# yxtay/glove-tensorflow

Measured on AMD Instinct MI355X. Metric: co-occurrence nonzeros/sec, higher is better.
Workload: dtype f32; 1 GPU; zipf_v400k_d300; V=400000, d=300, optimizer=Adagrad, batch_size_per_gpu=1048576, global_batch=1048576, nnz_per_gpu=25000000, chunk_cap=32, parallelism=single GPU, index=dealt

## Files before the change

### glove-tensorflow_amd/csrc/glove_epoch.hip

```cpp
#include "glove_common.h"

#include <type_traits>

namespace glove {

constexpr int kCsThreads = 256;
constexpr int kCsWaves = kCsThreads / 64;
constexpr int kCsMaxDigits = 2048;
constexpr int kCsMaxBits = 11;

struct CsGeom {
    int64_t n;
    int ntiles;
    int nd[2], db[2];
    int stride;
    uint32_t *count, *offs;
    uint32_t *tot;
};

template <int E, class Job>
__global__ __launch_bounds__(kCsThreads) void csort_hist(Job job, CsGeom g)
{
    __shared__ int hist[kCsMaxDigits];
    const int side = blockIdx.y, nd = g.nd[side], db = g.db[side];
// ... 7 lines not shown
#pragma unroll
        for (int j = 0; j < E; ++j) {
            const int64_t i = base + j * 64 + lane;
            if (i < g.n) { walk[j * kCsThreads + threadIdx.x] = job.position(side, i); cnt = j + 1; }
        }
        int j = 0;
        uint32_t x = cnt > 0 ? walk[threadIdx.x] : 0u;
        while (j < cnt) {
            x = job.seat_once(x);
            if (job.seated(x)) {
                walk[j * kCsThreads + threadIdx.x] = x;
                ++j;
                if (j < cnt) x = walk[j * kCsThreads + threadIdx.x];
            }
        }
    }
#pragma unroll 4
    for (int j = 0; j < E; ++j) {
        const int64_t i = base + j * 64 + lane;
        const bool valid = i < g.n;
        int digit = 0;
        if (Job::kSeats) { if (valid) digit = job.digit_of_seat(side, i, walk[j * kCsThreads + threadIdx.x]); }
        else if (valid) digit = job.digit(side, i);
        const unsigned long long peers = digit_peers(digit, db, valid);
        if (valid && lane == __ffsll((long long)peers) - 1) atomicAdd(&hist[digit], __popcll(peers));
    }
    __syncthreads();
    uint32_t *out = g.count + (size_t)side * g.stride * g.ntiles + blockIdx.x;
    for (int i = threadIdx.x; i < nd; i += kCsThreads) out[(size_t)i * g.ntiles] = (uint32_t)hist[i];
}

__device__ inline int block_excl_scan(int v, int *wtot , int &total)
{
    const int lane = threadIdx.x & 63, wave = threadIdx.x >> 6;
    int incl = v;
#pragma unroll
    for (int dlt = 1; dlt < 64; dlt <<= 1) {
        const int o = __shfl_up(incl, dlt, 64);
        if (lane >= dlt) incl += o;
    }
    __syncthreads();
    if (lane == 63) wtot[wave] = incl;
    __syncthreads();
    int start = incl - v;
    total = 0;
#pragma unroll
    for (int wv = 0; wv < kCsWaves; ++wv) {
        if (wv < wave) start += wtot[wv];
        total += wtot[wv];
    }
    return start;
}

__global__ __launch_bounds__(kCsThreads) void csort_scan(CsGeom g)
{
    __shared__ int wtot[kCsWaves];
    const int side = blockIdx.y, d = blockIdx.x;
    if (d >= g.nd[side]) return;
    const uint32_t *row = g.count + ((size_t)side * g.stride + d) * g.ntiles;
    uint32_t *out = g.offs + ((size_t)side * g.stride + d) * g.ntiles;
    constexpr int kPer = 8;
    int carry = 0;
    for (int base = 0; base < g.ntiles; base += kCsThreads * kPer) {
        int v[kPer], s = 0;
#pragma unroll
        for (int k = 0; k < kPer; ++k) {
            const int t = base + threadIdx.x * kPer + k;
            v[k] = t < g.ntiles ? (int)row[t] : 0;
            s += v[k];
        }
        int total;
        int run = carry + block_excl_scan(s, wtot, total);
#pragma unroll
        for (int k = 0; k < kPer; ++k) {
            const int t = base + threadIdx.x * kPer + k;
            if (t < g.ntiles) out[t] = (uint32_t)run;
            run += v[k];
        }
        carry += total;
    }
    if (threadIdx.x == 0) g.tot[(size_t)side * g.stride + d] = (uint32_t)carry;
}

template <int E, class Job>
__global__ __launch_bounds__(kCsThreads) void csort_scatter(Job job, CsGeom g)
{
    using Item = typename Job::Item;
    constexpr int T = kCsThreads * E;
    extern __shared__ __attribute__((aligned(16))) unsigned char cs_smem[];
    const int side = blockIdx.y, nd = g.nd[side], db = g.db[side];
    Item *stage = reinterpret_cast<Item *>(cs_smem);
    uint16_t *sdig = reinterpret_cast<uint16_t *>(stage + T);
    int *wcnt = reinterpret_cast<int *>(sdig + T);
    int *gbase = wcnt + kCsWaves * nd;
    int *tstart = gbase + nd;
    __shared__ int wtot[kCsWaves];
    const int lane = threadIdx.x & 63, wave = threadIdx.x >> 6;
    const int64_t tile0 = (int64_t)blockIdx.x * T;
    const int64_t base = tile0 + (int64_t)wave * (64 * E);
    Item it[E];
    int digit[E], rank[E];
#pragma unroll
    for (int j = 0; j < E; ++j) {
        const int64_t i = base + j * 64 + lane;
        digit[j] = 0;
        if (i < g.n) digit[j] = job.load(side, i, it[j]);
    }
    int *mine = wcnt + wave * nd;
    for (int i = lane; i < nd; i += 64) mine[i] = 0;
#pragma unroll
    for (int j = 0; j < E; ++j) {
        const bool valid = base + j * 64 + lane < g.n;
        const unsigned long long peers = digit_peers(digit[j], db, valid);
        const int leader = valid ? __ffsll((long long)peers) - 1 : lane;
        int before = 0;
        if (valid && lane == leader) before = atomicAdd(&mine[digit[j]], __popcll(peers));
        before = __shfl(before, leader, 64);
        rank[j] = before + __popcll(peers & ((1ull << lane) - 1ull));
    }
    __syncthreads();
    constexpr int kPer = kCsMaxDigits / kCsThreads;
    {
        const uint32_t *tot = g.tot + (size_t)side * g.stride;
        const uint32_t *offs = g.offs + (size_t)side * g.stride * g.ntiles + blockIdx.x;
        int tile_n[kPer], all_n[kPer], st = 0, sa = 0;
#pragma unroll
        for (int k = 0; k < kPer; ++k) {
            const int d = threadIdx.x * kPer + k;
            tile_n[k] = all_n[k] = 0;
            if (d < nd) {
                int run = 0;
#pragma unroll
                for (int wv = 0; wv < kCsWaves; ++wv) {
                    const int c = wcnt[wv * nd + d];
                    wcnt[wv * nd + d] = run;
                    run += c;
                }
                tile_n[k] = run;
                all_n[k] = (int)tot[d];
            }
            st += tile_n[k];
            sa += all_n[k];
        }
        int total;
        int ts = block_excl_scan(st, wtot, total);
        int ds = block_excl_scan(sa, wtot, total);
#pragma unroll
        for (int k = 0; k < kPer; ++k) {
            const int d = threadIdx.x * kPer + k;
            if (d < nd) {
                tstart[d] = ts;
                gbase[d] = ds + (int)offs[(size_t)d * g.ntiles] - ts;
            }
            ts += tile_n[k];
            ds += all_n[k];
        }
    }
    __syncthreads();
#pragma unroll
    for (int j = 0; j < E; ++j) {
        if (base + j * 64 + lane >= g.n) continue;
        const int lp = tstart[digit[j]] + mine[digit[j]] + rank[j];
        stage[lp] = it[j];
        sdig[lp] = (uint16_t)digit[j];
    }
    __syncthreads();
    const int64_t left = g.n - tile0;
    const int count = left < T ? (int)left : T;
#pragma unroll 4
    for (int k = 0; k < E; ++k) {
        const int lp = k * kCsThreads + threadIdx.x;
        if (lp >= count) break;
        job.store(side, (int64_t)(gbase[sdig[lp]] + lp), stage[lp]);
    }
}

struct CsWs {
    uint32_t *count, *offs, *tot;
    int ntiles, e;
    size_t bytes;
};

static int cs_e_for(int stride) { (void)stride; return 8; }

static CsWs carve_cs(void *ws, int64_t n, int stride)
{
    CsWs c;
    char *base = (char *)ws;
    size_t off = 0;
    auto take = [&](size_t bytes) { void *q = base + off; off += align_up(bytes, 256); return q; };
    c.e = cs_e_for(stride);
    const int64_t per_tile = (int64_t)kCsThreads * c.e;
    c.ntiles = (int)((n + per_tile - 1) / per_tile);
    if (c.ntiles < 1) c.ntiles = 1;
    c.count = (uint32_t *)take((size_t)2 * c.ntiles * stride * 4);
    c.offs = (uint32_t *)take((size_t)2 * c.ntiles * stride * 4);
    c.tot = (uint32_t *)take((size_t)2 * stride * 4);
    c.bytes = off;
    return c;
}

template <int E, class Job>
static int launch_cs_pass(const Job &job, const CsGeom &g, hipStream_t st)
{
    const size_t smem = (size_t)kCsThreads * E * (sizeof(typename Job::Item) + 2) + (size_t)(kCsWaves + 2) * g.stride * 4;
    hipError_t e = hipFuncSetAttribute(reinterpret_cast<const void *>(csort_scatter<E, Job>), hipFuncAttributeMaxDynamicSharedMemorySize, (int)smem);
    if (e != hipSuccess) return (int)e;
    hipLaunchKernelGGL((csort_hist<E, Job>), dim3(g.ntiles, 2), dim3(kCsThreads), 0, st, job, g);
    hipLaunchKernelGGL(csort_scan, dim3(g.stride, 2), dim3(kCsThreads), 0, st, g);
    hipLaunchKernelGGL((csort_scatter<E, Job>), dim3(g.ntiles, 2), dim3(kCsThreads), smem, st, job, g);
    return (int)hipGetLastError();
}

template <class Job>
static int run_cs_pass(const Job &job, const CsWs &c, int64_t n, const int (&db)[2], hipStream_t st)
{
    CsGeom g;
    g.n = n;
    g.ntiles = c.ntiles;
    for (int sd = 0; sd < 2; ++sd) { g.db[sd] = db[sd]; g.nd[sd] = 1 << db[sd]; }
    g.stride = g.nd[0] > g.nd[1] ? g.nd[0] : g.nd[1];
    g.count = c.count; g.offs = c.offs; g.tot = c.tot;
    return c.e == 16 ? launch_cs_pass<16, Job>(job, g, st) : launch_cs_pass<8, Job>(job, g, st);
}

static int ceil_log2_64(int64_t v)
{
    int b = 1;
    while (b < 62 && (1ll << b) < v) ++b;
    return b;
}

struct DealSide {
    const int32_t *id, *partner;
    const float *w, *y;
    const int32_t *link;
    int32_t *o_id, *o_partner;
    float *o_w, *o_y;
    int32_t *cache;
    int4 *tmp_pay;
    int32_t *tmp_batch;
};

struct DealItemLast { int32_t id, partner, w, y; };
struct DealItemMid { int32_t id, partner, w, y, batch; };

template <bool FIRST, bool LAST>
struct DealJob {
    DealSide s[2];
    uint64_t n;
    uint32_t B;
    int bits;
    uint4 key;
    int shift;
    uint32_t mask;
    int bshift;
    int nt;
    int cache8;
    using Item = typename std::conditional<LAST, DealItemLast, DealItemMid>::type;

    static constexpr bool kSeats = FIRST;
    __device__ uint32_t position(int side, int64_t i) const { return s[side].link ? (uint32_t)s[side].link[i] : (uint32_t)i; }
    __device__ uint32_t seat_once(uint32_t x) const { return feistel_once(x, bits, key); }
    __device__ bool seated(uint32_t x) const { return x < (uint32_t)n; }
    __device__ int digit_of_seat(int side, int64_t i, uint32_t seat) const
    {
        const int32_t batch = (int32_t)(bshift >= 0 ? seat >> bshift : seat / B);
        if (cache8) reinterpret_cast<uint8_t *>(s[side].cache)[i] = (uint8_t)batch; else s[side].cache[i] = batch;
        return (int)(((uint32_t)batch >> shift) & mask);
    }
    __device__ int digit(int side, int64_t i) const
    {
        if (FIRST) return digit_of_seat(side, i, feistel_walk(position(side, i), (uint32_t)n, bits, key));
        return (int)(((uint32_t)s[side].tmp_batch[i] >> shift) & mask);
    }
    __device__ int load(int side, int64_t i, Item &it) const
    {
        const DealSide &sd = s[side];
        int32_t batch;
        if (FIRST) {
            if (nt) {
                it.id = __builtin_nontemporal_load(sd.id + i); it.partner = __builtin_nontemporal_load(sd.partner + i);
                it.w = __float_as_int(__builtin_nontemporal_load(sd.w + i)); it.y = __float_as_int(__builtin_nontemporal_load(sd.y + i));
                batch = cache8 ? (int32_t)__builtin_nontemporal_load(reinterpret_cast<const uint8_t *>(sd.cache) + i) : __builtin_nontemporal_load(sd.cache + i);
            } else {
                it.id = sd.id[i]; it.partner = sd.partner[i];
                it.w = __float_as_int(sd.w[i]); it.y = __float_as_int(sd.y[i]);
                batch = cache8 ? (int32_t)reinterpret_cast<const uint8_t *>(sd.cache)[i] : sd.cache[i];
            }
        } else {
            const int4 v = sd.tmp_pay[i];
            it.id = v.x; it.partner = v.y; it.w = v.z; it.y = v.w;
            batch = sd.tmp_batch[i];
        }
        set_batch(it, batch);
        return (int)(((uint32_t)batch >> shift) & mask);
    }
    __device__ static void set_batch(DealItemLast &, int32_t) {}
    __device__ static void set_batch(DealItemMid &it, int32_t b) { it.batch = b; }
    __device__ void store(int side, int64_t dest, const DealItemLast &it) const
    {
        const DealSide &sd = s[side];
        if (nt) {
            __builtin_nontemporal_store(it.id, sd.o_id + dest); __builtin_nontemporal_store(it.partner, sd.o_partner + dest);
            __builtin_nontemporal_store(__int_as_float(it.w), sd.o_w + dest); __builtin_nontemporal_store(__int_as_float(it.y), sd.o_y + dest);
        } else {
            sd.o_id[dest] = it.id; sd.o_partner[dest] = it.partner;
            sd.o_w[dest] = __int_as_float(it.w); sd.o_y[dest] = __int_as_float(it.y);
        }
    }
    __device__ void store(int side, int64_t dest, const DealItemMid &it) const
    {
        const DealSide &sd = s[side];
        sd.tmp_pay[dest] = make_int4(it.id, it.partner, it.w, it.y);
        sd.tmp_batch[dest] = it.batch;
    }
};

struct DealPlan { int passes, db[2]; int64_t nb; };
static DealPlan deal_plan(int64_t n, int64_t B)
{
    DealPlan p;
    p.nb = (n + B - 1) / B;
    const int bits = ceil_log2_64(p.nb > 1 ? p.nb : 2);
    p.passes = bits <= kCsMaxBits ? 1 : 2;
    p.db[0] = p.passes == 1 ? bits : (bits + 1) / 2;
    p.db[1] = p.passes == 1 ? 0 : bits - p.db[0];
    return p;
}

struct DealWs { CsWs cs; int32_t *cache[2]; int4 *pay[2]; int32_t *batch[2]; size_t bytes; };
static DealWs carve_deal(void *ws, int64_t n, int64_t B)
{
    const DealPlan p = deal_plan(n, B);
    DealWs d;
    const int stride = 1 << (p.db[0] > p.db[1] ? p.db[0] : p.db[1]);
    d.cs = carve_cs(ws, n, stride);
    size_t off = d.cs.bytes;
    char *base = (char *)ws;
    auto take = [&](size_t bytes) { void *q = base + off; off += align_up(bytes, 256); return q; };
    for (int sd = 0; sd < 2; ++sd) {
        d.cache[sd] = (int32_t *)take((size_t)n * 4);
        d.pay[sd] = p.passes > 1 ? (int4 *)take((size_t)n * 16) : nullptr;
        d.batch[sd] = p.passes > 1 ? (int32_t *)take((size_t)n * 4) : nullptr;
    }
    d.bytes = off;
    return d;
}

struct MasterSide {
    const int32_t *major, *minor;
    uint32_t major_below, minor_below;
    const uint64_t *k_in; uint64_t *k_out;
    const int32_t *i_in; int32_t *i_out;
    int32_t *o_id, *o_partner, *o_perm;
    int shift;
    uint32_t mask;
};

template <bool FIRST, bool LAST>
struct MasterJob {
    MasterSide s[2];
    struct Item { uint64_t key; int32_t idx; };
    __device__ uint64_t key_of(int side, int64_t i) const
    {
        const MasterSide &sd = s[side];
        if (!FIRST) return sd.k_in[i];
        uint32_t a = (uint32_t)sd.major[i], b = (uint32_t)sd.minor[i];
        if (a >= sd.major_below) a = 0;
        if (b >= sd.minor_below) b = 0;
        return (uint64_t)a << 32 | b;
    }
    static constexpr bool kSeats = false;
    __device__ uint32_t position(int, int64_t) const { return 0u; }
    __device__ uint32_t seat_once(uint32_t x) const { return x; }
    __device__ bool seated(uint32_t) const { return true; }
    __device__ int digit_of_seat(int, int64_t, uint32_t) const { return 0; }
    __device__ int digit(int side, int64_t i) const { return (int)((uint32_t)(key_of(side, i) >> s[side].shift) & s[side].mask); }
    __device__ int load(int side, int64_t i, Item &it) const
    {
        it.key = key_of(side, i);
        it.idx = FIRST ? (int32_t)i : s[side].i_in[i];
        return (int)((uint32_t)(it.key >> s[side].shift) & s[side].mask);
    }
    __device__ void store(int side, int64_t dest, const Item &it) const
    {
        const MasterSide &sd = s[side];
        if (LAST) {
            sd.o_id[dest] = (int32_t)(it.key >> 32);
            sd.o_partner[dest] = (int32_t)(uint32_t)it.key;
            sd.o_perm[dest] = it.idx;
        } else {
            sd.k_out[dest] = it.key;
            sd.i_out[dest] = it.idx;
        }
    }
};

__global__ __launch_bounds__(kBlock) void masters_gather_kernel(const float *__restrict__ w, const float *__restrict__ y,
                                                                const int32_t *__restrict__ row, const int32_t *__restrict__ col,
                                                                uint32_t row_below, uint32_t col_below, int64_t n,
                                                                const int32_t *__restrict__ perm_r, const int32_t *__restrict__ perm_c,
                                                                float *__restrict__ w_r, float *__restrict__ y_r,
                                                                float *__restrict__ w_c, float *__restrict__ y_c,
                                                                int32_t *__restrict__ inv_r, int32_t *__restrict__ mapped)
{
    int bad = 0;
    for (int64_t k = (int64_t)blockIdx.x * kBlock + threadIdx.x; k < n; k += (int64_t)gridDim.x * kBlock) {
        const int32_t pr = perm_r[k], pc = perm_c[k];
        w_r[k] = w[pr]; y_r[k] = y[pr];
        w_c[k] = w[pc]; y_c[k] = y[pc];
        inv_r[pr] = (int32_t)k;
        bad += ((uint32_t)row[k] >= row_below) + ((uint32_t)col[k] >= col_below);
    }
    bad = wave_sum_int(bad);
    if (mapped && (threadIdx.x & 63) == 0 && bad) atomicAdd(mapped, bad);
}

__global__ __launch_bounds__(kBlock) void masters_link_kernel(const int32_t *__restrict__ perm_c, const int32_t *__restrict__ inv_r,
                                                              int64_t n, int32_t *__restrict__ link)
{
    for (int64_t q = (int64_t)blockIdx.x * kBlock + threadIdx.x; q < n; q += (int64_t)gridDim.x * kBlock) link[q] = inv_r[perm_c[q]];
}

struct MastersWs { CsWs cs; uint64_t *key[2][2]; int32_t *idx[2][2]; int32_t *perm[2]; int32_t *inv; size_t bytes; };
static MastersWs carve_masters(void *ws, int64_t n)
{
    MastersWs m;
    m.cs = carve_cs(ws, n, kCsMaxDigits);
    size_t off = m.cs.bytes;
    char *base = (char *)ws;
    auto take = [&](size_t bytes) { void *q = base + off; off += align_up(bytes, 256); return q; };
    const size_t nn = (size_t)(n > 0 ? n : 1);
    for (int sd = 0; sd < 2; ++sd)
        for (int i = 0; i < 2; ++i) {
            m.key[sd][i] = (uint64_t *)take(nn * 8);
            m.idx[sd][i] = (int32_t *)take(nn * 4);
        }
    for (int sd = 0; sd < 2; ++sd) m.perm[sd] = (int32_t *)take(nn * 4);
    m.inv = (int32_t *)take(nn * 4);
    m.bytes = off;
    return m;
}

static bool pairs_ok(const glove_pairs *p) { return p && p->id && p->partner && p->w && p->y; }

}

using namespace glove;

extern "C" {

size_t glove_masters_workspace_bytes(int64_t n)
{
    if (n < 0) return 0;
    return carve_masters(nullptr, n).bytes;
// ... 98 lines not shown
```

### glove-tensorflow_amd/csrc/glove_plan.hip

```cpp
#include "glove_common.h"

#include <cstring>

namespace glove {

constexpr int kSmallPlanMax = 4096;
int plan_build_small(const int32_t *row, const int32_t *col, const float *w, const float *y, int64_t B, int32_t V,
                     const PlanSet &set, int n, hipStream_t st);

constexpr int kSortThreads = 256;
constexpr int kSortWaves = kSortThreads / 64;
constexpr int kMaxDigits = 256;
constexpr int kWalk = 16;

struct SortSide {
    const int32_t *keys;
    const int32_t *vals;
    int32_t clean_below;
    int32_t *out_keys, *out_vals;
    int32_t *sorted_keys;
    const int32_t *other;
    int32_t other_below;
    int32_t *partner;
    float *w_out, *y_out;
// ... 169 lines not shown
        }
    }
    __syncthreads();
#pragma unroll
    for (int j = 0; j < E; ++j) {
        const int64_t i = base + j * 64 + lane;
        if (i >= in.n) continue;
        const int digit = (key[j] >> in.shift) & (nd - 1);
        const int dest = wcnt[wave][digit] + rank[j];
        const int32_t p = val[j];
        if (!LAST) {
            sd.out_keys[dest] = key[j];
            sd.out_vals[dest] = p;
        } else {
            sd.sorted_keys[dest] = key[j];
            int32_t o = g_id[j];
            if ((uint32_t)o >= (uint32_t)sd.other_below) o = 0;
            sd.partner[dest] = o;
            sd.w_out[dest] = g_w[j];
            sd.y_out[dest] = g_y[j];
            if (sd.where) { if (side == 0) sd.where[p] = dest; else sd.where[dest] = p; }
        }
    }
}


#define SIDE(x) (side ? x[1] : x[0])

constexpr int kTileThreads = 256;
constexpr int kTilePer = 8;
constexpr int kTile = kTileThreads * kTilePer;

struct SideKeys { const int32_t *keys[2]; };
struct SideOut {
    int32_t *chunk_id[2], *chunk_start[2], *uniq_slot[2];
    int32_t *counts;
    int32_t *uniq_rec[2];
    const int64_t *tile_re;
    int32_t *heavy;
    int heavy_chunks, cap_heavy;
    int2 *chunk_aux[2];
    uint32_t *mark[2];
    int mark_words[2];
    uint32_t *chunk_hw[2];
};

__device__ inline void tile_flags(const int32_t *__restrict__ keys, int64_t B, int64_t begin, int32_t chunk_cap,
                                  int64_t first_run_start, unsigned (&flag)[kTilePer], int &nu, int &nc, int64_t *lds_rs)
{
    const int64_t k0 = begin + (int64_t)threadIdx.x * kTilePer;
    int32_t key[kTilePer + 1];
    key[0] = (k0 > 0 && k0 <= B) ? keys[k0 - 1] : -1;
#pragma unroll
    for (int i = 0; i < kTilePer; ++i) key[i + 1] = (k0 + i < B) ? keys[k0 + i] : -1;
    int64_t my_last_start = -1;
#pragma unroll
    for (int i = 0; i < kTilePer; ++i) {
        const int64_t k = k0 + i;
        if (k < B && (k == 0 || key[i + 1] != key[i])) my_last_start = k;
    }
    const int lane = threadIdx.x & 63, wave = threadIdx.x >> 6;
    int64_t incl = my_last_start;
#pragma unroll
    for (int dlt = 1; dlt < 64; dlt <<= 1) {
        const int64_t o = __shfl_up(incl, dlt, 64);
        if (lane >= dlt) incl = o > incl ? o : incl;
    }
    if (lane == 63) lds_rs[wave] = incl;
    __syncthreads();
    int64_t carry = first_run_start;
    for (int wv = 0; wv < wave; ++wv) carry = lds_rs[wv] > carry ? lds_rs[wv] : carry;
    int64_t prev = __shfl_up(incl, 1, 64);
    if (lane == 0) prev = -1;
    int64_t run_start = prev > carry ? prev : carry;
    __syncthreads();
    nu = nc = 0;
#pragma unroll
    for (int i = 0; i < kTilePer; ++i) {
        const int64_t k = k0 + i;
        flag[i] = 0;
        if (k >= B) continue;
        const bool uniq = (k == 0 || key[i + 1] != key[i]);
        if (uniq) run_start = k;
        const bool chunk = uniq || ((int)(k - run_start) % chunk_cap == 0);
        flag[i] = (chunk ? 1u : 0u) | (uniq ? 2u : 0u);
        nu += uniq;
        nc += chunk;
    }
}

__device__ inline int64_t run_start_of(const int32_t *__restrict__ keys, int64_t pos)
{
    const int lane = threadIdx.x & 63;
    const int32_t key = keys[pos];
    int64_t lo = 0, hi = pos;
    if (pos > 0) {
        const int64_t q = pos - 1 - lane;
        const bool other = q >= 0 && keys[q] != key;
        const unsigned long long m = __ballot(other);
        if (m != 0) return pos - (__ffsll((long long)m) - 1);
        if (pos < 64) return 0;
        hi = pos - 64;
    }
    while (lo < hi) {
        const int64_t n = hi - lo, step = (n + 63) / 64;
        int64_t q = lo + step * lane;
        if (q > hi - 1) q = hi - 1;
        const bool ge = keys[q] >= key;
        const unsigned long long m = __ballot(ge);
        if (m == 0) {
            lo = __shfl(q, 63, 64) + 1;
            continue;
        }
        const int first = __ffsll((long long)m) - 1;
        const int64_t q_first = __shfl(q, first, 64);
        const int64_t q_before = __shfl(q, first > 0 ? first - 1 : 0, 64);
        lo = first == 0 ? lo : q_before + 1;
        hi = first == 0 ? lo : q_first;
    }
    return lo;
}

__device__ inline int64_t run_end_of(const int32_t *__restrict__ keys, int64_t B, int64_t pos)
{
    const int lane = threadIdx.x & 63;
    const int32_t key = keys[pos];
    int64_t lo = pos + 1, hi = B;
    {
        const int64_t q = pos + 1 + lane;
        const bool other = q < B && keys[q] != key;
        const unsigned long long m = __ballot(other);
        if (m != 0) return pos + 1 + (__ffsll((long long)m) - 1);
        if (pos + 65 >= B) return B;
        lo = pos + 65;
    }
    while (lo < hi) {
        const int64_t n = hi - lo, step = (n + 63) / 64;
        int64_t q = lo + step * lane;
        if (q > hi - 1) q = hi - 1;
        const bool gt = keys[q] > key;
        const unsigned long long m = __ballot(gt);
        if (m == 0) {
            lo = __shfl(q, 63, 64) + 1;
            continue;
        }
        const int first = __ffsll((long long)m) - 1;
        const int64_t q_first = __shfl(q, first, 64);
        const int64_t q_before = __shfl(q, first > 0 ? first - 1 : 0, 64);
        lo = first == 0 ? lo : q_before + 1;
        hi = first == 0 ? lo : q_first;
    }
    return lo;
}

struct TileExtra {
    int64_t *tile_re;
    int32_t *counts;
    const int32_t *mapped;
    int n_mapped;
    const int32_t *c_orig;
    const int32_t *rpos;
    int32_t *c_perm, *r_to_c;
};

struct SideCopy {
    const int32_t *p_src[2]; const float *w_src[2], *y_src[2];
    int32_t *p_dst[2]; float *w_dst[2], *y_dst[2];
};

struct SideOne {
    SideKeys sk;
    int64_t *tile_rs;
    int2 *tile_sums;
    TileExtra ex;
    SideOut out;
    SideCopy cp;
};
struct SideSet { SideOne b[kPlanSetMax]; };
__device__ inline const SideOne &pick(const SideOne &a) { return a; }
__device__ inline const SideOne &pick(const SideSet &a) { return a.b[blockIdx.z]; }

struct SortedSrc { const int32_t *id[2], *partner[2]; const float *w[2], *y[2]; };
struct SortedWs { char *base; size_t per_batch, tile_rs, tile_re, tile_sums, aux0, aux1; };
struct SideDev {
    const glove_plan *plans;
    SortedSrc src;
    SortedWs ws;
    int64_t B;
    int ntiles;
    int32_t V;
};
__device__ inline SideOne pick(const SideDev &a)
{
    const glove_plan &pl = a.plans[blockIdx.z];
    const size_t at = (size_t)blockIdx.z * (size_t)a.B;
    char *w = a.ws.base + (size_t)blockIdx.z * a.ws.per_batch;
    SideOne o;
    o.sk = SideKeys{{a.src.id[0] + at, a.src.id[1] + at}};
    o.tile_rs = reinterpret_cast<int64_t *>(w + a.ws.tile_rs);
    o.tile_sums = reinterpret_cast<int2 *>(w + a.ws.tile_sums);
    int64_t *tile_re = reinterpret_cast<int64_t *>(w + a.ws.tile_re);
    int2 *aux0 = reinterpret_cast<int2 *>(w + a.ws.aux0), *aux1 = reinterpret_cast<int2 *>(w + a.ws.aux1);
    o.ex = TileExtra{tile_re, pl.counts, nullptr, 0, nullptr, nullptr, nullptr, nullptr};
    o.out = SideOut{{pl.r_chunk_id, pl.c_chunk_id}, {pl.r_chunk_start, pl.c_chunk_start}, {pl.r_uniq_slot, pl.c_uniq_slot},
                    pl.counts, {pl.r_uniq_rec, pl.c_uniq_rec}, tile_re, pl.heavy, pl.heavy_chunks, pl.cap_heavy,
                    {pl.r_crec ? aux0 : nullptr, pl.r_crec ? aux1 : nullptr},
                    {pl.r_mark, pl.c_mark}, {((pl.V_row > 0 ? pl.V_row : a.V) + 31) / 32, (a.V + 31) / 32},
                    {pl.r_chunk_hw, pl.c_chunk_hw}};
    o.cp = SideCopy{{a.src.partner[0] + at, a.src.partner[1] + at}, {a.src.w[0] + at, a.src.w[1] + at}, {a.src.y[0] + at, a.src.y[1] + at},
                    {pl.r_partner, pl.c_partner}, {pl.r_w, pl.c_w}, {pl.r_y, pl.c_y}};
    return o;
}

template <class Args>
__global__ __launch_bounds__(kTileThreads) void side_tiles(Args args, int64_t B, int32_t chunk_cap, int ntiles)
{
    const SideOne &one = pick(args);
    const SideKeys &sk = one.sk;
    int64_t *__restrict__ tile_rs = one.tile_rs;
    int2 *__restrict__ tile_sums = one.tile_sums;
    const TileExtra &ex = one.ex;
    __shared__ int64_t lds_rs[kTileThreads / 64 + 1];
    __shared__ int red[2][kTileThreads / 64];
    const int side = blockIdx.y, t = blockIdx.x;
    const int32_t *keys = SIDE(sk.keys);
    const int64_t begin = (int64_t)t * kTile;
    if (SIDE(one.out.mark)) {
        uint32_t *mk = SIDE(one.out.mark);
        const int words = SIDE(one.out.mark_words);
        for (int i = t * kTileThreads + (int)threadIdx.x; i < words; i += ntiles * kTileThreads) mk[i] = 0u;
    }
    if (SIDE(one.cp.p_dst)) {
        const SideCopy &cp = one.cp;
        for (int64_t k = begin + threadIdx.x; k < begin + kTile && k < B; k += kTileThreads) {
            SIDE(cp.p_dst)[k] = SIDE(cp.p_src)[k];
            SIDE(cp.w_dst)[k] = SIDE(cp.w_src)[k];
            SIDE(cp.y_dst)[k] = SIDE(cp.y_src)[k];
        }
    }
    if (side == 1 && ex.c_perm) {
        const int64_t q0 = begin + (int64_t)threadIdx.x * kTilePer;
        int32_t o[kTilePer], rp[kTilePer];
#pragma unroll
        for (int i = 0; i < kTilePer; ++i) o[i] = q0 + i < B ? ex.c_orig[q0 + i] : 0;
#pragma unroll
        for (int i = 0; i < kTilePer; ++i) rp[i] = ex.rpos[o[i]];
#pragma unroll
        for (int i = 0; i < kTilePer; ++i) {
            if (q0 + i >= B) continue;
            ex.c_perm[q0 + i] = rp[i];
            ex.r_to_c[rp[i]] = (int32_t)(q0 + i);
        }
    }
    if (threadIdx.x < 64) {
        const int64_t r = begin > 0 ? run_start_of(keys, begin) : 0;
        if (threadIdx.x == 0) lds_rs[kTileThreads / 64] = r;
    } else if (threadIdx.x < 128) {
        const int64_t end = begin + kTile < B ? begin + kTile : B;
        const int64_t r = end < B ? run_end_of(keys, B, end - 1) : B;
        if (threadIdx.x == 64) ex.tile_re[(size_t)side * ntiles + t] = r;
    }
    __syncthreads();
    const int64_t frs = lds_rs[kTileThreads / 64];
    unsigned flag[kTilePer];
    int nu, nc;
    tile_flags(keys, B, begin, chunk_cap, frs, flag, nu, nc, lds_rs);
    nu = wave_sum_int(nu);
    nc = wave_sum_int(nc);
    if ((threadIdx.x & 63) == 0) { red[0][threadIdx.x >> 6] = nu; red[1][threadIdx.x >> 6] = nc; }
    __syncthreads();
    if (threadIdx.x == 0) {
        int su = 0, sc = 0;
        for (int wv = 0; wv < kTileThreads / 64; ++wv) { su += red[0][wv]; sc += red[1][wv]; }
        tile_sums[(size_t)side * ntiles + t] = make_int2(su, sc);
        tile_rs[(size_t)side * ntiles + t] = frs;
    }
    if (t == 0 && side == 0) {
        int v = 0;
        for (int i = threadIdx.x; i < ex.n_mapped; i += kTileThreads) v += ex.mapped[i];
        v = wave_sum_int(v);
        __syncthreads();
        if ((threadIdx.x & 63) == 0) red[0][threadIdx.x >> 6] = v;
        __syncthreads();
        if (threadIdx.x == 0) {
            int total = 0;
            for (int wv = 0; wv < kTileThreads / 64; ++wv) total += red[0][wv];
            ex.counts[5] = total;
            ex.counts[4] = ex.counts[6] = ex.counts[7] = 0;
        }
    }
}

template <class Args>
__global__ __launch_bounds__(kTileThreads) void side_emit(Args args, int64_t B, int32_t chunk_cap, int ntiles)
{
    const SideOne &one = pick(args);
    const SideKeys &sk = one.sk;
    const int64_t *__restrict__ tile_rs = one.tile_rs;
    const int2 *__restrict__ tile_sums = one.tile_sums;
    const SideOut &out = one.out;
    __shared__ int64_t lds_rs[kTileThreads / 64 + 1];
    __shared__ int64_t lds_open[kTileThreads / 64];
    __shared__ int red[2][kTileThreads / 64];
    __shared__ int wave_tot[2][kTileThreads / 64];
    const int side = blockIdx.y, t = blockIdx.x;
    const int32_t *keys = SIDE(sk.keys);
    const int64_t begin = (int64_t)t * kTile;
    int pu = 0, pc = 0;
    for (int i = threadIdx.x; i < t; i += kTileThreads) {
        const int2 v = tile_sums[(size_t)side * ntiles + i];
        pu += v.x;
        pc += v.y;
    }
    pu = wave_sum_int(pu);
    pc = wave_sum_int(pc);
    if ((threadIdx.x & 63) == 0) { red[0][threadIdx.x >> 6] = pu; red[1][threadIdx.x >> 6] = pc; }
    __syncthreads();
    int base_u = 0, base_c = 0;
    for (int wv = 0; wv < kTileThreads / 64; ++wv) { base_u += red[0][wv]; base_c += red[1][wv]; }
    unsigned flag[kTilePer];
    int nu, nc;
    tile_flags(keys, B, begin, chunk_cap, tile_rs[(size_t)side * ntiles + t], flag, nu, nc, lds_rs);
    const int lane = threadIdx.x & 63, wave = threadIdx.x >> 6;
    int iu = nu, ic = nc;
#pragma unroll
    for (int dlt = 1; dlt < 64; dlt <<= 1) {
        const int ou = __shfl_up(iu, dlt, 64), oc = __shfl_up(ic, dlt, 64);
        if (lane >= dlt) { iu += ou; ic += oc; }
    }
    if (lane == 63) { wave_tot[0][wave] = iu; wave_tot[1][wave] = ic; }
    __syncthreads();
    int ui = base_u + iu - nu, ci = base_c + ic - nc;
    for (int wv = 0; wv < wave; ++wv) { ui += wave_tot[0][wv]; ci += wave_tot[1][wv]; }
    const int64_t k0 = begin + (int64_t)threadIdx.x * kTilePer;
    int32_t *chunk_id = SIDE(out.chunk_id), *chunk_start = SIDE(out.chunk_start), *uniq_slot = SIDE(out.uniq_slot);
    int open_ui[kTilePer], open_ci[kTilePer];
    int64_t my_first_open = INT64_MAX;
#pragma unroll
    for (int i = kTilePer - 1; i >= 0; --i)
        if (flag[i] & 2u) my_first_open = k0 + i;
#pragma unroll
    for (int i = 0; i < kTilePer; ++i) {
        const int64_t k = k0 + i;
        open_ui[i] = ui;
        open_ci[i] = ci;
        if (flag[i] & 2u) uniq_slot[ui++] = ci;
        if (flag[i] & 1u) { chunk_id[ci] = keys[k]; chunk_start[ci] = (int32_t)k; ++ci; }
        if (k == B - 1) {
            chunk_start[ci] = (int32_t)B;
            uniq_slot[ui] = ci;
            out.counts[2 * side] = ci;
            out.counts[2 * side + 1] = ui;
        }
    }
    int64_t sfx = my_first_open;
#pragma unroll
    for (int dlt = 1; dlt < 64; dlt <<= 1) {
        const int64_t o = __shfl_down(sfx, dlt, 64);
        if (lane + dlt < 64) sfx = o < sfx ? o : sfx;
    }
    if (lane == 0) lds_open[wave] = sfx;
    __syncthreads();
    int64_t next_open = out.tile_re[(size_t)side * ntiles + t];
    for (int wv = kTileThreads / 64 - 1; wv > wave; --wv) next_open = lds_open[wv] < next_open ? lds_open[wv] : next_open;
    int64_t right = __shfl_down(sfx, 1, 64);
    if (lane == 63) right = INT64_MAX;
    next_open = right < next_open ? right : next_open;
    int2 *aux = SIDE(out.chunk_aux);
#pragma unroll
    for (int i = kTilePer - 1; i >= 0; --i) {
        if (!(flag[i] & 1u)) continue;
        const int64_t k = k0 + i;
        const int pairs = (int)(next_open - k), chunks = (pairs + chunk_cap - 1) / chunk_cap;
        if (aux || SIDE(out.chunk_hw)) {
            const bool opens = (flag[i] & 2u) != 0;
            const uint32_t hw = (uint32_t)(chunks - 1) | (opens ? 0x80000000u : 0u);
            if (aux) aux[open_ci[i]] = make_int2(opens ? open_ui[i] : open_ui[i] - 1, (int)hw);
            if (SIDE(out.chunk_hw)) SIDE(out.chunk_hw)[open_ci[i]] = hw;
        }
        if (!(flag[i] & 2u)) continue;
        reinterpret_cast<int4 *>(SIDE(out.uniq_rec))[open_ui[i]] = make_int4(keys[k], open_ci[i], chunks, pairs);
        if (SIDE(out.mark)) atomicOr(SIDE(out.mark) + (keys[k] >> 5), 1u << (keys[k] & 31));
        if (chunks > out.heavy_chunks) {
            const int slot = atomicAdd(out.counts + 4, 1);
            if (slot < out.cap_heavy) out.heavy[slot] = (side << 30) | open_ui[i];
        }
        next_open = k;
    }
}

struct RecordArgs {
    const int32_t *uniq_slot[2];
    const int32_t *chunk_id[2], *chunk_start[2], *partner[2];
    const float *w[2], *y[2];
    int32_t *crec[2];
    const int2 *chunk_aux[2];
    int header_in_record;
};
struct RecordOne { RecordArgs a; const int32_t *counts; };
struct RecordSet { RecordOne b[kPlanSetMax]; };
__device__ inline const RecordOne &pick(const RecordOne &a) { return a; }
__device__ inline const RecordOne &pick(const RecordSet &a) { return a.b[blockIdx.z]; }
struct RecordDev { SideDev d; };
__device__ inline RecordOne pick(const RecordDev &r)
{
    const SideDev &a = r.d;
    const glove_plan &pl = a.plans[blockIdx.z];
    const size_t at = (size_t)blockIdx.z * (size_t)a.B;
    char *w = a.ws.base + (size_t)blockIdx.z * a.ws.per_batch;
    RecordOne o;
    o.a = RecordArgs{{pl.r_uniq_slot, pl.c_uniq_slot}, {pl.r_chunk_id, pl.c_chunk_id}, {pl.r_chunk_start, pl.c_chunk_start},
                     {a.src.partner[0] + at, a.src.partner[1] + at}, {a.src.w[0] + at, a.src.w[1] + at}, {a.src.y[0] + at, a.src.y[1] + at},
                     {pl.r_crec, pl.c_crec},
                     {reinterpret_cast<const int2 *>(w + a.ws.aux0), reinterpret_cast<const int2 *>(w + a.ws.aux1)}, 0};
    o.counts = pl.counts;
    return o;
}

typedef int v4i_t __attribute__((ext_vector_type(4)));

template <class Args>
__global__ __launch_bounds__(kBlock) void fill_records(Args args, int capP, int nt)
{
    const RecordOne &rone = pick(args);
    const RecordArgs &a = rone.a;
    const int32_t *__restrict__ counts = rone.counts;
    const int side = blockIdx.y;
    const int n_chunks = counts[2 * side];
    const int32_t *chunk_id = SIDE(a.chunk_id), *chunk_start = SIDE(a.chunk_start), *partner = SIDE(a.partner);
    const float *w = SIDE(a.w), *y = SIDE(a.y);
    const int2 *aux = SIDE(a.chunk_aux);
    const int sq = rec_stride_q(capP);
    const int lane = threadIdx.x & 63, g = lane & 7, oct = lane >> 3;
    const int j0 = (int)((blockIdx.x * (kBlock / 64) + (threadIdx.x >> 6)) * 32);
    if (j0 >= n_chunks) return;
    const int jl = j0 + lane < n_chunks ? j0 + lane : n_chunks;
    const int cs = lane <= 32 ? chunk_start[jl] : 0;
    constexpr int kStage = 384;
    __shared__ int32_t st_p[kBlock / 64][kStage];
    __shared__ float st_w[kBlock / 64][kStage], st_y[kBlock / 64][kStage];
    const int wv = threadIdx.x >> 6;
    const int p0 = __shfl(cs, 0, 64);
    const int last = n_chunks - j0 < 32 ? n_chunks - j0 : 32;
    const int span = __shfl(cs, last, 64) - p0;
    const bool staged = span <= kStage;
    if (staged) {
// ... 409 lines not shown
```

Measured before the change: 1.907 billion nonzeros/s.

## Defer item loads in deal scatter and derive run bounds from tile summaries

In the counting-sort scatter for the first-and-last deal pass, digits are now read from the cached batch array and the full 16-byte items are loaded only after ranks are known, in two halves, with 1-byte digit staging when few digits are used. This cuts register pressure and shared memory so more workgroups fit per CU. Separately, the chunk-planning kernels drop the per-tile binary searches for run start and end. They instead record each tile's first and last run opening and rebuild run bounds and chunk-count corrections with a max-scan over earlier tiles and a search for the next opening tile. That removes dependent global reads, but adds an O(tiles) prefix loop per block.

```diff
diff --git a/glove-tensorflow_amd/csrc/glove_epoch.hip b/glove-tensorflow_amd/csrc/glove_epoch.hip
--- a/glove-tensorflow_amd/csrc/glove_epoch.hip
+++ b/glove-tensorflow_amd/csrc/glove_epoch.hip
@@ -113,6 +113,15 @@
     if (threadIdx.x == 0) g.tot[(size_t)side * g.stride + d] = (uint32_t)carry;
 }
 
+template <class Job>
+__host__ __device__ constexpr int cs_sdig_bytes(int stride) { return Job::kDigitsCached && stride <= 256 ? 1 : 2; }
+template <int E, class Job>
+__host__ __device__ constexpr size_t cs_scatter_lds(int stride)
+{
+    return (size_t)kCsThreads * E * (sizeof(typename Job::Item) + cs_sdig_bytes<Job>(stride)) + (size_t)(kCsWaves + 2) * stride * 4;
+}
+constexpr size_t kCsLdsBesidePasses = (163840 - 3 * 30176) / 2;
+
 template <int E, class Job>
 __global__ __launch_bounds__(kCsThreads) void csort_scatter(Job job, CsGeom g)
 {
@@ -120,22 +129,25 @@
     constexpr int T = kCsThreads * E;
     extern __shared__ __attribute__((aligned(16))) unsigned char cs_smem[];
     const int side = blockIdx.y, nd = g.nd[side], db = g.db[side];
+    const bool dig8 = cs_sdig_bytes<Job>(g.stride) == 1;
     Item *stage = reinterpret_cast<Item *>(cs_smem);
     uint16_t *sdig = reinterpret_cast<uint16_t *>(stage + T);
-    int *wcnt = reinterpret_cast<int *>(sdig + T);
+    uint8_t *sdig8 = reinterpret_cast<uint8_t *>(stage + T);
+    int *wcnt = reinterpret_cast<int *>(dig8 ? (unsigned char *)(sdig8 + T) : (unsigned char *)(sdig + T));
     int *gbase = wcnt + kCsWaves * nd;
     int *tstart = gbase + nd;
     __shared__ int wtot[kCsWaves];
     const int lane = threadIdx.x & 63, wave = threadIdx.x >> 6;
     const int64_t tile0 = (int64_t)blockIdx.x * T;
     const int64_t base = tile0 + (int64_t)wave * (64 * E);
-    Item it[E];
+    Item it[Job::kDigitsCached ? 1 : E];
     int digit[E], rank[E];
 #pragma unroll
     for (int j = 0; j < E; ++j) {
         const int64_t i = base + j * 64 + lane;
         digit[j] = 0;
-        if (i < g.n) digit[j] = job.load(side, i, it[j]);
+        if constexpr (Job::kDigitsCached) { if (i < g.n) digit[j] = job.cached_digit(side, i); }
+        else if (i < g.n) digit[j] = job.load(side, i, it[j]);
     }
     int *mine = wcnt + wave * nd;
     for (int i = lane; i < nd; i += 64) mine[i] = 0;
@@ -188,12 +200,34 @@
         }
     }
     __syncthreads();
-#pragma unroll
-    for (int j = 0; j < E; ++j) {
-        if (base + j * 64 + lane >= g.n) continue;
-        const int lp = tstart[digit[j]] + mine[digit[j]] + rank[j];
-        stage[lp] = it[j];
-        sdig[lp] = (uint16_t)digit[j];
+    if constexpr (Job::kDigitsCached) {
+#pragma unroll
+        for (int j = 0; j < E; ++j) {
+            if (base + j * 64 + lane >= g.n) continue;
+            rank[j] += tstart[digit[j]] + mine[digit[j]];
+            if (dig8) sdig8[rank[j]] = (uint8_t)digit[j]; else sdig[rank[j]] = (uint16_t)digit[j];
+        }
+        constexpr int kHalf = E / 2;
+#pragma unroll
+        for (int r = 0; r < E; r += kHalf) {
+            Item part[kHalf];
+#pragma unroll
+            for (int j = 0; j < kHalf; ++j) {
+                const int64_t i = base + (r + j) * 64 + lane;
+                if (i < g.n) job.load_item(side, i, part[j]);
+            }
+#pragma unroll
+            for (int j = 0; j < kHalf; ++j)
+                if (base + (r + j) * 64 + lane < g.n) stage[rank[r + j]] = part[j];
+        }
+    } else {
+#pragma unroll
+        for (int j = 0; j < E; ++j) {
+            if (base + j * 64 + lane >= g.n) continue;
+            const int lp = tstart[digit[j]] + mine[digit[j]] + rank[j];
+            stage[lp] = it[j];
+            sdig[lp] = (uint16_t)digit[j];
+        }
     }
     __syncthreads();
     const int64_t left = g.n - tile0;
@@ -202,7 +236,8 @@
     for (int k = 0; k < E; ++k) {
         const int lp = k * kCsThreads + threadIdx.x;
         if (lp >= count) break;
-        job.store(side, (int64_t)(gbase[sdig[lp]] + lp), stage[lp]);
+        const int d = Job::kDigitsCached && dig8 ? (int)sdig8[lp] : (int)sdig[lp];
+        job.store(side, (int64_t)(gbase[d] + lp), stage[lp]);
     }
 }
 
@@ -234,7 +269,7 @@
 template <int E, class Job>
 static int launch_cs_pass(const Job &job, const CsGeom &g, hipStream_t st)
 {
-    const size_t smem = (size_t)kCsThreads * E * (sizeof(typename Job::Item) + 2) + (size_t)(kCsWaves + 2) * g.stride * 4;
+    const size_t smem = cs_scatter_lds<E, Job>(g.stride);
     hipError_t e = hipFuncSetAttribute(reinterpret_cast<const void *>(csort_scatter<E, Job>), hipFuncAttributeMaxDynamicSharedMemorySize, (int)smem);
     if (e != hipSuccess) return (int)e;
     hipLaunchKernelGGL((csort_hist<E, Job>), dim3(g.ntiles, 2), dim3(kCsThreads), 0, st, job, g);
@@ -305,6 +340,27 @@
         if (FIRST) return digit_of_seat(side, i, feistel_walk(position(side, i), (uint32_t)n, bits, key));
         return (int)(((uint32_t)s[side].tmp_batch[i] >> shift) & mask);
     }
+    static constexpr bool kDigitsCached = FIRST && LAST;
+    __device__ int cached_digit(int side, int64_t i) const
+    {
+        const DealSide &sd = s[side];
+        int32_t batch;
+        if (nt) batch = cache8 ? (int32_t)__builtin_nontemporal_load(reinterpret_cast<const uint8_t *>(sd.cache) + i) : __builtin_nontemporal_load(sd.cache + i);
+        else batch = cache8 ? (int32_t)reinterpret_cast<const uint8_t *>(sd.cache)[i] : sd.cache[i];
+        return (int)(((uint32_t)batch >> shift) & mask);
+    }
+    __device__ void load_item(int side, int64_t i, DealItemLast &it) const
+    {
+        const DealSide &sd = s[side];
+        if (nt) {
+            it.id = __builtin_nontemporal_load(sd.id + i); it.partner = __builtin_nontemporal_load(sd.partner + i);
+            it.w = __float_as_int(__builtin_nontemporal_load(sd.w + i)); it.y = __float_as_int(__builtin_nontemporal_load(sd.y + i));
+        } else {
+            it.id = sd.id[i]; it.partner = sd.partner[i];
+            it.w = __float_as_int(sd.w[i]); it.y = __float_as_int(sd.y[i]);
+        }
+    }
+    __device__ void load_item(int, int64_t, DealItemMid &) const {}
     __device__ int load(int side, int64_t i, Item &it) const
     {
         const DealSide &sd = s[side];
@@ -348,6 +404,11 @@
     }
 };
 
+static_assert(sizeof(DealItemLast) == 16, "a dealt pair is staged as 16 bytes");
+static_assert(cs_scatter_lds<8, DealJob<true, true>>(64) + kCsWaves * sizeof(int) <= kCsLdsBesidePasses,
+              "csort_scatter<8, DealJob<true, true>>: two workgroups no longer fit beside three pass workgroups");
+static_assert(cs_scatter_lds<8, DealJob<true, true>>(32) + kCsWaves * sizeof(int) == 35600, "LDS of the headline deal's scatter");
+
 struct DealPlan { int passes, db[2]; int64_t nb; };
 static DealPlan deal_plan(int64_t n, int64_t B)
 {
@@ -403,6 +464,9 @@
         return (uint64_t)a << 32 | b;
     }
     static constexpr bool kSeats = false;
+    static constexpr bool kDigitsCached = false;
+    __device__ int cached_digit(int, int64_t) const { return 0; }
+    __device__ void load_item(int, int64_t, Item &) const {}
     __device__ uint32_t position(int, int64_t) const { return 0u; }
     __device__ uint32_t seat_once(uint32_t x) const { return x; }
     __device__ bool seated(uint32_t) const { return true; }
diff --git a/glove-tensorflow_amd/csrc/glove_plan.hip b/glove-tensorflow_amd/csrc/glove_plan.hip
--- a/glove-tensorflow_amd/csrc/glove_plan.hip
+++ b/glove-tensorflow_amd/csrc/glove_plan.hip
@@ -275,75 +275,11 @@
         if (k >= B) continue;
         const bool uniq = (k == 0 || key[i + 1] != key[i]);
         if (uniq) run_start = k;
-        const bool chunk = uniq || ((int)(k - run_start) % chunk_cap == 0);
+        const bool chunk = uniq || (run_start >= 0 && (int)(k - run_start) % chunk_cap == 0);
         flag[i] = (chunk ? 1u : 0u) | (uniq ? 2u : 0u);
         nu += uniq;
         nc += chunk;
     }
-}
-
-__device__ inline int64_t run_start_of(const int32_t *__restrict__ keys, int64_t pos)
-{
-    const int lane = threadIdx.x & 63;
-    const int32_t key = keys[pos];
-    int64_t lo = 0, hi = pos;
-    if (pos > 0) {
-        const int64_t q = pos - 1 - lane;
-        const bool other = q >= 0 && keys[q] != key;
-        const unsigned long long m = __ballot(other);
-        if (m != 0) return pos - (__ffsll((long long)m) - 1);
-        if (pos < 64) return 0;
-        hi = pos - 64;
-    }
-    while (lo < hi) {
-        const int64_t n = hi - lo, step = (n + 63) / 64;
-        int64_t q = lo + step * lane;
-        if (q > hi - 1) q = hi - 1;
-        const bool ge = keys[q] >= key;
-        const unsigned long long m = __ballot(ge);
-        if (m == 0) {
-            lo = __shfl(q, 63, 64) + 1;
-            continue;
-        }
-        const int first = __ffsll((long long)m) - 1;
-        const int64_t q_first = __shfl(q, first, 64);
-        const int64_t q_before = __shfl(q, first > 0 ? first - 1 : 0, 64);
-        lo = first == 0 ? lo : q_before + 1;
-        hi = first == 0 ? lo : q_first;
-    }
-    return lo;
-}
-
-__device__ inline int64_t run_end_of(const int32_t *__restrict__ keys, int64_t B, int64_t pos)
-{
-    const int lane = threadIdx.x & 63;
-    const int32_t key = keys[pos];
-    int64_t lo = pos + 1, hi = B;
-    {
-        const int64_t q = pos + 1 + lane;
-        const bool other = q < B && keys[q] != key;
-        const unsigned long long m = __ballot(other);
-        if (m != 0) return pos + 1 + (__ffsll((long long)m) - 1);
-        if (pos + 65 >= B) return B;
-        lo = pos + 65;
-    }
-    while (lo < hi) {
-        const int64_t n = hi - lo, step = (n + 63) / 64;
-        int64_t q = lo + step * lane;
-        if (q > hi - 1) q = hi - 1;
-        const bool gt = keys[q] > key;
-        const unsigned long long m = __ballot(gt);
-        if (m == 0) {
-            lo = __shfl(q, 63, 64) + 1;
-            continue;
-        }
-        const int first = __ffsll((long long)m) - 1;
-        const int64_t q_first = __shfl(q, first, 64);
-        const int64_t q_before = __shfl(q, first > 0 ? first - 1 : 0, 64);
-        lo = first == 0 ? lo : q_before + 1;
-        hi = first == 0 ? lo : q_first;
-    }
-    return lo;
 }
 
 struct TileExtra {
@@ -414,6 +350,7 @@
     int2 *__restrict__ tile_sums = one.tile_sums;
     const TileExtra &ex = one.ex;
     __shared__ int64_t lds_rs[kTileThreads / 64 + 1];
+    __shared__ int64_t lds_fo[kTileThreads / 64];
     __shared__ int red[2][kTileThreads / 64];
     const int side = blockIdx.y, t = blockIdx.x;
     const int32_t *keys = SIDE(sk.keys);
@@ -445,28 +382,36 @@
             ex.r_to_c[rp[i]] = (int32_t)(q0 + i);
         }
     }
-    if (threadIdx.x < 64) {
-        const int64_t r = begin > 0 ? run_start_of(keys, begin) : 0;
-        if (threadIdx.x == 0) lds_rs[kTileThreads / 64] = r;
-    } else if (threadIdx.x < 128) {
-        const int64_t end = begin + kTile < B ? begin + kTile : B;
-        const int64_t r = end < B ? run_end_of(keys, B, end - 1) : B;
-        if (threadIdx.x == 64) ex.tile_re[(size_t)side * ntiles + t] = r;
-    }
-    __syncthreads();
-    const int64_t frs = lds_rs[kTileThreads / 64];
     unsigned flag[kTilePer];
     int nu, nc;
-    tile_flags(keys, B, begin, chunk_cap, frs, flag, nu, nc, lds_rs);
+    tile_flags(keys, B, begin, chunk_cap, -1, flag, nu, nc, lds_rs);
+    const int64_t k0 = begin + (int64_t)threadIdx.x * kTilePer;
+    int64_t fo = INT64_MAX;
+#pragma unroll
+    for (int i = kTilePer - 1; i >= 0; --i)
+        if (flag[i] & 2u) fo = k0 + i;
+#pragma unroll
+    for (int dlt = 32; dlt > 0; dlt >>= 1) {
+        const int64_t o = __shfl_xor(fo, dlt, 64);
+        fo = o < fo ? o : fo;
+    }
     nu = wave_sum_int(nu);
     nc = wave_sum_int(nc);
-    if ((threadIdx.x & 63) == 0) { red[0][threadIdx.x >> 6] = nu; red[1][threadIdx.x >> 6] = nc; }
+    if ((threadIdx.x & 63) == 0) { red[0][threadIdx.x >> 6] = nu; red[1][threadIdx.x >> 6] = nc; lds_fo[threadIdx.x >> 6] = fo; }
     __syncthreads();
     if (threadIdx.x == 0) {
         int su = 0, sc = 0;
-        for (int wv = 0; wv < kTileThreads / 64; ++wv) { su += red[0][wv]; sc += red[1][wv]; }
+        const int64_t end = begin + kTile < B ? begin + kTile : B;
+        int64_t first = end, last = -1;
+        for (int wv = 0; wv < kTileThreads / 64; ++wv) {
+            su += red[0][wv];
+            sc += red[1][wv];
+            first = lds_fo[wv] < first ? lds_fo[wv] : first;
+            last = lds_rs[wv] > last ? lds_rs[wv] : last;
+        }
         tile_sums[(size_t)side * ntiles + t] = make_int2(su, sc);
-        tile_rs[(size_t)side * ntiles + t] = frs;
+        tile_rs[(size_t)side * ntiles + t] = first;
+        ex.tile_re[(size_t)side * ntiles + t] = last;
     }
     if (t == 0 && side == 0) {
         int v = 0;
@@ -496,25 +441,72 @@
     __shared__ int64_t lds_open[kTileThreads / 64];
     __shared__ int red[2][kTileThreads / 64];
     __shared__ int wave_tot[2][kTileThreads / 64];
+    __shared__ int scan_max[kTileThreads / 64];
     const int side = blockIdx.y, t = blockIdx.x;
     const int32_t *keys = SIDE(sk.keys);
     const int64_t begin = (int64_t)t * kTile;
-    int pu = 0, pc = 0;
-    for (int i = threadIdx.x; i < t; i += kTileThreads) {
-        const int2 v = tile_sums[(size_t)side * ntiles + i];
-        pu += v.x;
-        pc += v.y;
+    const int lane = threadIdx.x & 63, wave = threadIdx.x >> 6;
+    const int64_t *__restrict__ first_open = tile_rs + (size_t)side * ntiles;
+    const int64_t *__restrict__ last_open = out.tile_re + (size_t)side * ntiles;
+    int pu = 0, pc = 0, carry = 0;
+    for (int r0 = 0; r0 < t; r0 += kTileThreads) {
+        const int i = r0 + (int)threadIdx.x;
+        const bool in = i < t;
+        const int2 v = in ? tile_sums[(size_t)side * ntiles + i] : make_int2(0, 0);
+        const int lo = in ? (int)last_open[i] : -1, fo = in ? (int)first_open[i] : 0;
+        int incl = lo;
+#pragma unroll
+        for (int dlt = 1; dlt < 64; dlt <<= 1) {
+            const int o = __shfl_up(incl, dlt, 64);
+            if (lane >= dlt) incl = o > incl ? o : incl;
+        }
+        __syncthreads();
+        if (lane == 63) scan_max[wave] = incl;
+        __syncthreads();
+        int s = __shfl_up(incl, 1, 64);
+        if (lane == 0) s = -1;
+        s = carry > s ? carry : s;
+#pragma unroll
+        for (int wv = 0; wv < kTileThreads / 64; ++wv) {
+            const int m = scan_max[wv];
+            if (wv < wave) s = m > s ? m : s;
+            carry = m > carry ? m : carry;
+        }
+        if (in) {
+            const uint32_t cap = (uint32_t)chunk_cap, b = (uint32_t)i * (uint32_t)kTile;
+            pu += v.x;
+            pc += v.y + (int)(((uint32_t)(fo - s) + cap - 1u) / cap - ((b - (uint32_t)s) + cap - 1u) / cap);
+        }
+    }
+    const int64_t frs = carry;
+    int64_t run_end = B;
+    for (int r0 = t + 1; r0 < ntiles; r0 += kTileThreads) {
+        const int i = r0 + (int)threadIdx.x;
+        int64_t fo = INT64_MAX;
+        if (i < ntiles) {
+            const int64_t f = first_open[i], e = (int64_t)(i + 1) * kTile;
+            if (f < (e < B ? e : B)) fo = f;
+        }
+        const unsigned long long m = __ballot(fo != INT64_MAX);
+        const int64_t wmin = __shfl(fo, m ? __ffsll((long long)m) - 1 : 0, 64);
+        __syncthreads();
+        if (lane == 0) lds_open[wave] = wmin;
+        __syncthreads();
+        int64_t found = INT64_MAX;
+#pragma unroll
+        for (int wv = kTileThreads / 64 - 1; wv >= 0; --wv) found = lds_open[wv] < found ? lds_open[wv] : found;
+        if (found != INT64_MAX) { run_end = found; break; }
     }
     pu = wave_sum_int(pu);
     pc = wave_sum_int(pc);
-    if ((threadIdx.x & 63) == 0) { red[0][threadIdx.x >> 6] = pu; red[1][threadIdx.x >> 6] = pc; }
+    __syncthreads();
+    if (lane == 0) { red[0][wave] = pu; red[1][wave] = pc; }
     __syncthreads();
     int base_u = 0, base_c = 0;
     for (int wv = 0; wv < kTileThreads / 64; ++wv) { base_u += red[0][wv]; base_c += red[1][wv]; }
     unsigned flag[kTilePer];
     int nu, nc;
-    tile_flags(keys, B, begin, chunk_cap, tile_rs[(size_t)side * ntiles + t], flag, nu, nc, lds_rs);
-    const int lane = threadIdx.x & 63, wave = threadIdx.x >> 6;
+    tile_flags(keys, B, begin, chunk_cap, frs, flag, nu, nc, lds_rs);
     int iu = nu, ic = nc;
 #pragma unroll
     for (int dlt = 1; dlt < 64; dlt <<= 1) {
@@ -554,7 +546,7 @@
     }
     if (lane == 0) lds_open[wave] = sfx;
     __syncthreads();
-    int64_t next_open = out.tile_re[(size_t)side * ntiles + t];
+    int64_t next_open = run_end;
     for (int wv = kTileThreads / 64 - 1; wv > wave; --wv) next_open = lds_open[wv] < next_open ? lds_open[wv] : next_open;
     int64_t right = __shfl_down(sfx, 1, 64);
     if (lane == 63) right = INT64_MAX;
```

After: 1.845 billion nonzeros/s. 3.2% lower.
